# Hydr10n/DirectX-Raytracing-Spheres-Demo

Hardware: AMD Instinct MI355X
Metric: Mrays/s (CastRay-equivalents incl. primaries) at 1920x1080, 8 bounces, 1 spp (higher is better)
Workload: dtype f32

## Files before the change

directx-raytracing-spheres-demo_amd/csrc/pt_api.hip:

```cpp
#include <hip/hip_runtime.h>
#include <rccl/rccl.h>
#include <dlfcn.h>
#include <link.h>

#include <algorithm>
#include <chrono>
#include <cmath>
#include <cstdio>
#include <cstdlib>
#include <cstring>
#include <new>
#include <string>
#include <limits>
#include <vector>

#include "../../include/pt_api.h"
#include "pt_kernels.h"
#include "pt_beam_cache.h"
#include "pt_bloom.h"
#include "pt_nrd.h"
#include "pt_denoise.h"
#include "pt_lbvh.h"
#include "pt_lbvh_gpu.h"

using namespace pt;

namespace {

constexpr uint32_t kMaxLdsBytes = 160u * 1024u;
constexpr uint32_t kSahMaxSpheres = 4096u;
constexpr uint32_t kLdsSceneBudget = 64u * 1024u;

struct EventPair {
    hipEvent_t a, b;
    int kind;
};

}

struct Knobs {
    int split = -1, traverse_blocks_per_cu = -1, fused_threads = -1, no_adaptive_grid = -1, shade_blocks_per_cu = -1, tail_threshold = -1,
        tail_blocks_per_cu = -1, loop_threads = -1, inline2_min_slots = -1, tail_after = -1, seg = -1, loop_use_tail = -1, fuse_loop = -1,
        ray_replacement = -1, dyn_blocks_per_cu = -1, debug_counts = -1, sah = -1, sah_max_spheres = -1, beams = -1, wide = -1, descent = -1, roctx = -1, lane_priority = -1, fused_refit = -1, beam_reach = -1, beam_max_slack_pct = -1, beam_max_margin = -1, beam_share_wgs = -1, refl_beams = -1;
};

struct Lane {
    hipStream_t stream = nullptr;
    hipEvent_t ev_done = nullptr;
    size_t cap_slots = 0;
    RayQueue q[2]{};
    Scratch scratch{};
    bool scratch_spp = false;
    uint32_t* d_counts = nullptr;
    size_t cap_counts = 0;
    uint32_t parity = 0;
    uint32_t* h_counts = nullptr;
    uint32_t* h_prev_counts = nullptr;
    uint32_t* d_prev_counts = nullptr;
    uint64_t prev_signature = 0;
    uint32_t* d_seg_counts = nullptr;
    static constexpr uint32_t kTotals = 10;
    unsigned long long* d_totals = nullptr;
    float4* d_sph = nullptr;
    float4* d_sph_sorted = nullptr;
    float4* d_nodes = nullptr;
    uint32_t* d_refit_flags = nullptr;
    uint32_t* d_refit_hdr = nullptr;
    PtSphere* h_stage = nullptr;
    const float4* d_stage = nullptr;
    hipEvent_t ev_upload = nullptr;
    hipEvent_t ev_poll[4] = {};
    uint32_t scene_n = 0;
    bool scene_private = false;
    uint64_t sph_gen = 0;
    bool needs_refit = false;
    bool upload_pending = false;
    const void* last_out = nullptr;
    const void* last_dn[3] = {};
    const void* last_di[2] = {};
    float4* d_rot = nullptr;
    float4* h_rot_stage = nullptr;
    hipEvent_t ev_rot = nullptr;
    uint64_t rot_gen = 0;
    uint32_t rot_n = 0;
    float4* d_prev_pose = nullptr;
    float4* h_prev_stage = nullptr;
    hipEvent_t ev_prev = nullptr;
    uint32_t prev_cap = 0;
    hipEvent_t ev_gb_in = nullptr;
    void* last_gb[13] = {};
};
constexpr uint32_t kMaxLanes = 8;

struct PtContext {
    int device = 0;
    hipStream_t stream = nullptr;
    bool own_stream = false;
    uint32_t flags = 0;
    uint32_t tile_size = 32;
    uint32_t num_cus = 256;
    Knobs knobs;
    std::string err;
// ... 172 lines not shown
        r.handle = dlopen(name, RTLD_NOW | RTLD_LOCAL);
    }
    if (!r.handle) { r.error = std::string("cannot load librccl.so: ") + dlerror(); return r; }
    auto sym = [&](const char* n) { void* p = dlsym(r.handle, n); if (!p && r.error.empty()) r.error = std::string("librccl.so lacks ") + n; return p; };
    r.GetUniqueId = reinterpret_cast<decltype(r.GetUniqueId)>(sym("ncclGetUniqueId"));
    r.CommInitRank = reinterpret_cast<decltype(r.CommInitRank)>(sym("ncclCommInitRank"));
    r.CommDestroy = reinterpret_cast<decltype(r.CommDestroy)>(sym("ncclCommDestroy"));
    r.GroupStart = reinterpret_cast<decltype(r.GroupStart)>(sym("ncclGroupStart"));
    r.GroupEnd = reinterpret_cast<decltype(r.GroupEnd)>(sym("ncclGroupEnd"));
    r.Send = reinterpret_cast<decltype(r.Send)>(sym("ncclSend"));
    r.Recv = reinterpret_cast<decltype(r.Recv)>(sym("ncclRecv"));
    r.GetErrorString = reinterpret_cast<decltype(r.GetErrorString)>(sym("ncclGetErrorString"));
    if (!r.error.empty()) { dlclose(r.handle); r.handle = nullptr; }
    return r;
}

PtStatus fail(PtContext* ctx, PtStatus st, const std::string& msg)
{
    if (ctx) ctx->err = msg;
    return st;
}

#define PT_HIP(ctx, expr)                                                                              \
    do {                                                                                               \
        hipError_t e_ = (expr);                                                                        \
        if (e_ != hipSuccess) {                                                                        \
            return fail(ctx, e_ == hipErrorOutOfMemory ? PT_ERR_OOM : PT_ERR_HIP,                      \
                        std::string(#expr) + ": " + hipGetErrorString(e_));                            \
        }                                                                                              \
    } while (0)

template <typename T>
void free_dev(T*& p)
{
    if (p) { (void)hipFree(p); p = nullptr; }
}

void free_lane_scene(Lane& L)
{
    free_dev(L.d_sph); free_dev(L.d_sph_sorted); free_dev(L.d_nodes); free_dev(L.d_refit_flags); free_dev(L.d_refit_hdr);
    if (L.h_stage) { (void)hipHostFree(L.h_stage); L.h_stage = nullptr; L.d_stage = nullptr; }
    L.scene_n = 0;
    L.scene_private = false;
    L.upload_pending = false;
    L.needs_refit = false;
}

void free_lane_buffers(Lane& L)
{
    for (auto& q : L.q) { free_dev(q.q0); free_dev(q.q1); free_dev(q.q2); free_dev(q.hit); }
    free_dev(L.scratch.sample_rad); free_dev(L.scratch.radiance); free_dev(L.scratch.primary_hit); free_dev(L.scratch.di); free_dev(L.scratch.primary_cache);
    free_dev(L.scratch.dn.rec); free_dev(L.scratch.dn.di_s);
    L.cap_slots = 0;
    L.scratch_spp = false;
}

PtStatus ensure_buffers(PtContext* c, Lane& L, size_t n_slots, bool need_spp, bool need_hits, size_t n_counts, bool need_di = false)
{
    if (n_slots > L.cap_slots || (need_hits && !L.q[0].hit)) {
        PT_HIP(c, hipStreamSynchronize(L.stream));
        free_lane_buffers(L);
        for (auto& q : L.q) {
            PT_HIP(c, hipMalloc(&q.q0, n_slots * sizeof(float4)));
            PT_HIP(c, hipMalloc(&q.q1, n_slots * sizeof(float4)));
            PT_HIP(c, hipMalloc(&q.q2, n_slots * sizeof(float4)));
            if (need_hits) PT_HIP(c, hipMalloc(&q.hit, n_slots * sizeof(uint2)));
        }
        PT_HIP(c, hipMalloc(&L.scratch.sample_rad, n_slots * sizeof(float4)));
        L.cap_slots = n_slots;
    }
    if (need_di && !L.scratch.di) PT_HIP(c, hipMalloc(&L.scratch.di, L.cap_slots * sizeof(float4)));
    if ((need_spp || need_di) && !L.scratch.primary_hit) PT_HIP(c, hipMalloc(&L.scratch.primary_hit, L.cap_slots * sizeof(uint2)));
    if (need_spp && !L.scratch_spp) {
        PT_HIP(c, hipMalloc(&L.scratch.radiance, L.cap_slots * sizeof(float4)));
        PT_HIP(c, hipMalloc(&L.scratch.primary_cache, L.cap_slots * 3u * sizeof(float4)));
        L.scratch_spp = true;
    }
    if (n_counts > L.cap_counts) {
        free_dev(L.d_counts);
        if (L.h_counts) { (void)hipHostFree(L.h_counts); L.h_counts = nullptr; }
        if (L.h_prev_counts) { (void)hipHostFree(L.h_prev_counts); L.h_prev_counts = nullptr; }
        PT_HIP(c, hipHostMalloc(&L.h_prev_counts, n_counts * sizeof(uint32_t), hipHostMallocMapped));
        std::memset(L.h_prev_counts, 0, n_counts * sizeof(uint32_t));
        PT_HIP(c, hipHostGetDevicePointer(reinterpret_cast<void**>(&L.d_prev_counts), L.h_prev_counts, 0));
        L.prev_signature = 0;
        PT_HIP(c, hipMalloc(&L.d_counts, 4 * n_counts * sizeof(uint32_t)));
        PT_HIP(c, hipMemsetAsync(L.d_counts, 0, 4 * n_counts * sizeof(uint32_t), L.stream));
        PT_HIP(c, hipHostMalloc(&L.h_counts, n_counts * sizeof(uint32_t)));
        L.cap_counts = n_counts;
    }
    return PT_OK;
}

hipError_t sync_all(PtContext* c)
{
    for (uint32_t i = 0; i < c->n_lanes; i++)
        if (c->lanes[i].stream) { hipError_t e = hipStreamSynchronize(c->lanes[i].stream); if (e != hipSuccess) return e; }
    if (c->beam.stream) { hipError_t e = hipStreamSynchronize(c->beam.stream); if (e != hipSuccess) return e; }
    return c->stream ? hipStreamSynchronize(c->stream) : hipSuccess;
}

void free_textures(PtContext* c)
{
    for (auto& img : c->d_tex_images) free_dev(img);
    c->d_tex_images.clear();
    c->tex_dims.clear();
    free_dev(c->d_tex); free_dev(c->d_tex_maps); free_dev(c->d_rot);
    c->has_textures = false;
}

PtStatus sync_lane_rotations(PtContext* c, Lane& L)
{
    if (!c->has_textures || c->rot_gen == c->rot_master_gen || (L.rot_gen == c->rot_gen && L.rot_n == c->n)) return PT_OK;
    const uint32_t n = c->n;
    if (L.rot_n != n) {
        PT_HIP(c, hipStreamSynchronize(L.stream));
        free_dev(L.d_rot);
        if (L.h_rot_stage) { (void)hipHostFree(L.h_rot_stage); L.h_rot_stage = nullptr; }
        PT_HIP(c, hipMalloc(&L.d_rot, (size_t)n * sizeof(float4)));
        PT_HIP(c, hipHostMalloc(&L.h_rot_stage, (size_t)n * sizeof(float4)));
        if (!L.ev_rot) PT_HIP(c, hipEventCreateWithFlags(&L.ev_rot, hipEventDisableTiming));
        L.rot_n = n;
// ... 61 lines not shown
{
    SceneView sv{};
    const bool priv = L && L->scene_private;
    sv.nodes = priv ? L->d_nodes : c->d_nodes;
    sv.wide = priv ? nullptr : c->d_wide;
    sv.sph_sorted = priv ? L->d_sph_sorted : c->d_sph_sorted;
    sv.sorted_id = c->d_leaf_ids ? c->d_leaf_ids : c->d_sorted_id;
    sv.alpha_class = c->d_alpha_class;
    sv.alpha_tested = c->alpha_tested ? 1u : 0u;
    sv.sph = priv ? L->d_sph : c->d_sph;
    sv.mats = c->d_mats;
    sv.n = c->n;
    sv.n_nodes = c->n_nodes;
    sv.stack_depth = stack_entries(c, sv.wide != nullptr);
    sv.descent_cap = c->lds_scene ? 0u : knob_or(c->knobs.descent, 8u);
    sv.lds_scene = c->lds_scene ? 1u : 0u;
    for (int i = 0; i < 4; i++) sv.env[i] = c->sd.EnvironmentLightColor[i];
    if (c->has_textures) { sv.tex = c->d_tex; sv.tex_maps = c->d_tex_maps; sv.rot = (c->rot_gen != c->rot_master_gen && L && L->d_rot && L->rot_gen == c->rot_gen) ? L->d_rot : c->d_rot; }
    sv.env_tex = c->sd.EnvironmentLightTextureDescriptor;
    sv.env_cube = c->sd.IsEnvironmentLightTextureCubeMap ? 1u : 0u;
    for (int r = 0; r < 3; r++)
        for (int k = 0; k < 3; k++) sv.env_xf[3 * r + k] = c->sd.EnvironmentLightTransform[4 * r + k];
    sv.lights = c->d_lights; sv.n_lights = c->n_lights;
    return sv;
}

FrameParams make_frame_params(const PtContext* c)
{
    FrameParams fp{};
    fp.cam = camera_params(c->cam, c->gs.RenderSize[0], c->gs.RenderSize[1]);
    fp.frame_index = c->gs.FrameIndex;
    fp.bounces = c->gs.Bounces;
    fp.spp = c->gs.SamplesPerPixel;
    fp.rr_enabled = c->gs.IsRussianRouletteEnabled ? 1u : 0u;
    fp.throughput_threshold = c->gs.ThroughputThreshold;
    fp.inv_spp = 1.0f / (float)c->gs.SamplesPerPixel;
    fp.di_enabled = (c->gs.IsDIEnabled && c->n_lights > 0) ? 1u : 0u;
    return fp;
}

int env_knob(const char* name)
{
    const char* v = std::getenv(name);
    if (!v || !*v) return -1;
    return (int)std::strtoul(v, nullptr, 10);
}

Knobs read_knobs()
{
    Knobs k;
    k.split = env_knob("PT_SPLIT"); k.traverse_blocks_per_cu = env_knob("PT_TRAVERSE_BLOCKS_PER_CU"); k.fused_threads = env_knob("PT_FUSED_THREADS");
    k.no_adaptive_grid = std::getenv("PT_NO_ADAPTIVE_GRID") ? 1 : -1; k.shade_blocks_per_cu = env_knob("PT_SHADE_BLOCKS_PER_CU");
    k.tail_threshold = env_knob("PT_TAIL_THRESHOLD"); k.tail_blocks_per_cu = env_knob("PT_TAIL_BLOCKS_PER_CU"); k.loop_threads = env_knob("PT_LOOP_THREADS");
    k.inline2_min_slots = env_knob("PT_INLINE2_MIN_SLOTS"); k.tail_after = env_knob("PT_TAIL_AFTER"); k.seg = env_knob("PT_SEG");
    k.loop_use_tail = std::getenv("PT_LOOP_USE_TAIL") ? 1 : -1; k.fuse_loop = env_knob("PT_FUSE_LOOP"); k.beam_reach = env_knob("PT_BEAM_REACH"); k.beam_max_slack_pct = env_knob("PT_BEAM_MAX_SLACK_PCT"); k.beam_max_margin = env_knob("PT_BEAM_MAX_MARGIN"); k.beam_share_wgs = env_knob("PT_BEAM_SHARE_WGS"); k.lane_priority = env_knob("PT_LANE_PRIORITY"); k.fused_refit = env_knob("PT_FUSED_REFIT"); k.ray_replacement = env_knob("PT_RAY_REPLACEMENT");
    k.dyn_blocks_per_cu = env_knob("PT_DYN_BLOCKS_PER_CU"); k.debug_counts = std::getenv("PT_DEBUG_COUNTS") ? 1 : -1; k.sah = env_knob("PT_SAH");
    k.sah_max_spheres = env_knob("PT_SAH_MAX_SPHERES"); k.beams = env_knob("PT_BEAMS"); k.refl_beams = env_knob("PT_REFL_BEAMS"); k.wide = env_knob("PT_WIDE"); k.descent = env_knob("PT_DESCENT"); k.roctx = env_knob("PT_ROCTX");
    return k;
}

EventPair* next_events(PtContext* c, int kind)
{
    if (c->ev_used >= (1u << 20)) return nullptr;
    if (c->ev_used == c->ev_pool.size()) {
        EventPair p{};
        if (hipEventCreate(&p.a) != hipSuccess || hipEventCreate(&p.b) != hipSuccess) return nullptr;
        c->ev_pool.push_back(p);
    }
    EventPair* p = &c->ev_pool[c->ev_used++];
    p->kind = kind;
    return p;
}

uint64_t bytes_per_secondary(bool split) { return split ? 144ull : 96ull; }
uint64_t fixed_bytes(bool split, uint64_t slots, uint64_t pixels, uint64_t spp_paths)
{
    return (split ? 112ull * slots : 0ull) + 16ull * pixels + 48ull * spp_paths;
}

FrameCounters make_counters(const Lane& L, uint32_t parity)
{
    FrameCounters fc{};
    fc.counts = L.d_counts + (size_t)parity * 2 * L.cap_counts;
    fc.fold_counts = L.d_counts + (size_t)(parity ^ 1u) * 2 * L.cap_counts;
    fc.n_counts = (uint32_t)L.cap_counts - 1u;
    fc.tail_rays = L.d_totals + 2 + parity;
    fc.fold_tail = L.d_totals + 2 + (parity ^ 1u);
    fc.totals = L.d_totals;
    fc.host_counts = L.d_prev_counts;
    return fc;
}

hipError_t flush_all_counters(Lane& L)
{
    if (!L.d_counts) return hipSuccess;
    for (uint32_t i = 0; i < 2; i++) {
        const FrameCounters fc = make_counters(L, L.parity ^ 1u ^ i);
        hipError_t e = launch_flush_counters(fc.counts, fc.n_counts, fc.tail_rays, fc.totals, fc.host_counts, L.stream);
        if (e != hipSuccess) return e;
    }
    return hipSuccess;
}

void sum_events(PtContext* c, size_t begin, size_t end, PtStats* stats)
{
    for (size_t i = begin; i < end; i++) {
        float t = 0;
// ... 251 lines not shown
static PtStatus sync_lane_spheres(PtContext* c, Lane& L)
{
    if (c->latest_lane < 0 || L.sph_gen == c->sph_gen) return PT_OK;
    const Lane& src = c->lanes[c->latest_lane];
    if (PtStatus st = stage_spheres_on_lane(c, L, reinterpret_cast<const PtSphere*>(src.h_stage)); st != PT_OK) return st;
    L.sph_gen = c->sph_gen;
    return refit_lane(c, L);
}

static PtStatus check_environment(PtContext* c)
{
    if (const uint32_t env = c->sd.EnvironmentLightTextureDescriptor; env != ~0u) {
        const size_t n_faces = c->sd.IsEnvironmentLightTextureCubeMap ? 6 : 1;
        if (!c->has_textures || (size_t)env + n_faces > c->tex_dims.size())
            return fail(c, PT_ERR_STATE, "SceneData.EnvironmentLightTextureDescriptor names a texture the table of pt_set_textures does not hold (call pt_set_textures after pt_set_scene; a cube map takes six consecutive entries)");
        for (size_t f = 0; f < n_faces; f++)
            if (n_faces == 6 && (c->tex_dims[env + f].first != c->tex_dims[env].first || c->tex_dims[env + f].second != c->tex_dims[env].first))
                return fail(c, PT_ERR_STATE, "SceneData.EnvironmentLightTextureDescriptor: the six faces of a cube map must be square and of one size");
    }
    return PT_OK;
}

struct SuppliedDI {
    const float4* diffuse;
    const float4* specular;
};
PtStatus render_common(PtContext* c, const PixelMap& pm, uint64_t valid_pixels, float4* out, PtStats* stats, const DenoiseOut* dn = nullptr,
                       const SuppliedDI* ext = nullptr)
{
    const RoctxRange range(c, ext ? "pt_render_with_di" : (dn ? "pt_render_denoiser" : (pm.mode == 0 ? "pt_render" : "pt_render_tiles")));
    const uint32_t bounces = c->gs.Bounces, spp = c->gs.SamplesPerPixel;
    if (const PtStatus st = check_environment(c); st != PT_OK) return st;
    const size_t max_iters = (size_t)spp * bounces + 1;
    const size_t wf_cap = spp > 1 ? max_iters : std::min<size_t>(max_iters, 64);
    const bool split = (c->flags & PT_FLAG_SPLIT_KERNELS) || knob_or(c->knobs.split, c->lds_scene ? 0u : 1u) != 0;
    if (traverse_lds_bytes_for(c->n_nodes, c->n, stack_entries(c, c->d_wide != nullptr), c->lds_scene) > kMaxLdsBytes - 9u * 1024u)
        return fail(c, PT_ERR_UNSUPPORTED, "BVH depth needs more traversal-stack LDS than a workgroup can have");
    Lane& L = c->lanes[c->next_lane];
    if (wf_cap + 2 > L.cap_counts && L.cap_counts) {
        PT_HIP(c, flush_all_counters(L));
        PT_HIP(c, hipStreamSynchronize(L.stream));
    }
    const bool di = ext || (c->gs.IsDIEnabled && c->n_lights > 0);
    const bool gb_before = c->gb_frame == c->frames && c->gb_lane == c->next_lane;
    bool lanes_idle = !gb_before || c->gb_lanes_idle;
    for (uint32_t i = 0; i < c->n_lanes && lanes_idle; i++)
        if (!(gb_before && i == c->next_lane) && hipStreamQuery(c->lanes[i].stream) != hipSuccess) { lanes_idle = false; (void)hipGetLastError(); }
    const bool big_frame = c->lds_scene && pm.n_slots >= 1500000u;
    const uint32_t trav_cap = c->num_cus * knob_or(c->knobs.traverse_blocks_per_cu, big_frame ? 2 : 8);
    const uint32_t fused_threads = c->lds_scene ? knob_or(c->knobs.fused_threads, 512) : 256u;
    auto grid_for = [](uint32_t items, uint32_t threads, uint32_t cap) { return std::max(1u, std::min((items + threads - 1) / threads, cap)); };
    const uint32_t primary_grid = grid_for(pm.n_slots, fused_threads, trav_cap);
    const uint32_t primary_batches = (pm.n_slots + fused_threads - 1) / fused_threads;
    const uint32_t seg_cap = (primary_batches + primary_grid - 1) / primary_grid * fused_threads;
    const size_t seg_total = (size_t)primary_grid * seg_cap;
    const bool seg_possible = !split && max_iters > 1 && primary_grid <= kMaxSegs && knob_or(c->knobs.seg, 1u) != 0 && c->knobs.loop_use_tail < 0;
    PtStatus st = ensure_buffers(c, L, split ? pm.n_slots : std::max<size_t>(pm.n_slots, seg_total), spp > 1, split, wf_cap + 2, di);
    if (st != PT_OK) return st;
    if (dn && !L.scratch.dn.rec) PT_HIP(c, hipMalloc(&L.scratch.dn.rec, L.cap_slots * sizeof(float4)));
    if (dn && dn->mode != 1 && di && !L.scratch.dn.di_s) PT_HIP(c, hipMalloc(&L.scratch.dn.di_s, L.cap_slots * sizeof(float4)));
    if ((st = sync_lane_rotations(c, L)) != PT_OK) return st;
    if ((st = sync_lane_spheres(c, L)) != PT_OK) return st;
    if (L.needs_refit && (st = refit_lane(c, L)) != PT_OK) return st;
    c->last_lane = c->next_lane;
    c->next_lane = (c->next_lane + 1) % c->n_lanes;
    c->frames++;
    const uint32_t* beam_lists = nullptr;
    const uint32_t* refl_lists = nullptr;
    BeamJob beam_job{};
    if (!split && !L.scene_private && c->n_nodes > 0 && knob_or(c->knobs.beams, 1u) != 0 && std::fabs(c->cam.Jitter[0]) <= 0.5f && std::fabs(c->cam.Jitter[1]) <= 0.5f) {
        hipEvent_t beam_wait = nullptr;
        if ((st = beam_cache_lookup(c, pm, std::min(primary_grid, knob_or(c->knobs.beam_share_wgs, 128u)) * 64u, &beam_lists, &refl_lists, &beam_wait, &beam_job)) != PT_OK) return st;
        if (beam_wait) PT_HIP(c, hipStreamWaitEvent(L.stream, beam_wait, 0));
    } else {
        c->beam.last_key.clear();
        c->beam.inc.active = false;
    }
    if (L.stream != c->stream) {
        const uint64_t nl = c->n_lanes;
        PT_HIP(c, hipEventRecord(c->ev_in[c->calls % nl], c->stream));
        const hipEvent_t marker = c->ev_in[c->calls >= nl - 1 ? (c->calls - (nl - 1)) % nl : 0];
        if (hipEventQuery(marker) != hipSuccess) {
            (void)hipGetLastError();
            PT_HIP(c, hipStreamWaitEvent(L.stream, marker, 0));
        }
        const void* mine[4] = { out, dn ? dn->diffuse : nullptr, dn ? dn->specular : nullptr, dn ? dn->spec_hit_dist : nullptr };
        bool reused = false;
        for (uint32_t i = 0; i < c->n_lanes && !reused; i++) {
            if (&c->lanes[i] == &L) continue;
            const Lane& o = c->lanes[i];
            const void* theirs[6] = { o.last_out, o.last_dn[0], o.last_dn[1], o.last_dn[2], o.last_di[0], o.last_di[1] };
            for (int a = 0; a < 4 && !reused; a++)
                for (int b = 0; b < 6 && !reused; b++) reused = mine[a] && mine[a] == theirs[b];
        }
        if (ext) reused = true;
        if (reused) PT_HIP(c, hipStreamWaitEvent(L.stream, c->ev_in[c->calls % nl], 0));
        L.last_out = out;
        for (int a = 0; a < 3; a++) L.last_dn[a] = mine[a + 1];
        L.last_di[0] = ext ? ext->diffuse : nullptr;
        L.last_di[1] = ext ? ext->specular : nullptr;
        c->calls++;
    }

    const SceneView sv = make_scene_view(c, &L);
    Scratch scr = L.scratch;
    scr.dn = DenoiseOut{};
    if (dn) {
        scr.dn = *dn;
        scr.dn.rec = L.scratch.dn.rec;
        scr.dn.di_s = L.scratch.dn.di_s;
// ... 18 lines not shown
    const uint32_t shade_cap = c->num_cus * knob_or(c->knobs.shade_blocks_per_cu, 16);
    const bool loop_is_main = spp > 1 && !split && c->knobs.tail_threshold < 0;
    const uint32_t tail_cap = c->num_cus * knob_or(c->knobs.tail_blocks_per_cu, loop_is_main ? 2 : 8);
    const uint32_t trav_threads = traverse_threads(c->lds_scene);
    const uint32_t loop_threads = knob_or(c->knobs.loop_threads, c->lds_scene && (loop_is_main || big_frame) ? 512u : 256u);
    const bool inline2 = !split && spp == 1 && pm.n_slots >= knob_or(c->knobs.inline2_min_slots, 0u);
    const size_t tail_after = knob_or(c->knobs.tail_after, split ? 4 : (inline2 ? 0 : 1));
    const uint32_t tail_threshold = knob_or(c->knobs.tail_threshold, 262144);

    const bool timed = stats != nullptr;
    const size_t ev_begin = c->ev_used;
    if (timed) PT_HIP(c, hipEventRecord(c->ev0, L.stream));

    auto bracket = [&](int kind, auto&& launch) -> hipError_t {
        EventPair* ev = c->profiling ? next_events(c, kind) : nullptr;
        if (ev) (void)hipEventRecord(ev->a, L.stream);
        hipError_t e = launch();
        if (ev) (void)hipEventRecord(ev->b, L.stream);
        return e;
    };
    auto poll = [&](size_t k, bool& empty, bool& go_loop) -> PtStatus {
        empty = false;
        if (loop_is_main) {
            go_loop = true;
        } else if (spp > 1) {
            constexpr size_t kPollLag = 2;
            PT_HIP(c, hipMemcpyAsync(L.h_counts + k + 1, counts + k + 1, sizeof(uint32_t), hipMemcpyDeviceToHost, L.stream));
            PT_HIP(c, hipEventRecord(L.ev_poll[k & 3], L.stream));
            go_loop = k + 2 >= wf_cap;
            if (k >= kPollLag) {
                PT_HIP(c, hipEventSynchronize(L.ev_poll[(k - kPollLag) & 3]));
                const uint32_t v = L.h_counts[k - kPollLag + 1];
                empty = v == 0;
                go_loop = go_loop || v < tail_threshold;
            }
        } else {
            go_loop = k >= tail_after || k + 2 >= wf_cap;
        }
        return PT_OK;
    };

    auto submit = [&]() -> PtStatus {
        if (ext) {
            PT_HIP(c, bracket(1, [&] { return launch_di_gather(pm, ext->diffuse, ext->specular, L.scratch.di, scr.dn.mode > 1 ? scr.dn.di_s : nullptr, L.stream); }));
        } else if (fp.di_enabled && split) {
            const uint32_t di_grid = grid_for(pm.n_slots, trav_threads, trav_cap_wide);
            PT_HIP(c, bracket(1, [&] { return launch_di(sv, pm, fp, L.scratch.di, L.scratch.primary_hit, fc.tail_rays, di_grid, L.stream, scr.dn.mode > 1 ? scr.dn.di_s : nullptr); }));
        }
        if (!split) {
            const bool loop_follows_primary = loop_is_main || (spp == 1 && (tail_after == 0 || wf_cap <= 2));
            const bool seg = loop_follows_primary && seg_possible;
            FrameCounters fc_seg = fc;
            const bool fuse = seg && knob_or(c->knobs.fuse_loop, (pm.n_slots < 400000u || (lanes_idle && spp == 1)) ? 1u : 0u) != 0;
            if (seg) { fc_seg.seg_counts = L.d_seg_counts; fc_seg.n_segs = primary_grid; fc_seg.seg_cap = seg_cap; fc_seg.fuse_loop = fuse ? 1u : 0u; }
            Scratch scratch = scr;
            if (sv.tex_maps || fuse || spp == 1) scratch.primary_cache = nullptr;
            for (size_t k = 0;; k++) {
                const RayQueue& qin = L.q[k & 1];
                const RayQueue& qout = L.q[(k + 1) & 1];
                const bool primary = k == 0;
                bool go_loop = false, empty = false;
                if (k > 0) {
                    if ((st = poll(k - 1, empty, go_loop)) != PT_OK) return st;
                    if (empty) break;
                }
                const bool last_possible = k + 1 >= max_iters;
                const bool loop = (k > 0 && go_loop);
                const uint32_t threads = loop ? loop_threads : fused_threads;
                const uint32_t items = primary ? pm.n_slots : estimate(k);
                const uint32_t cap = loop ? tail_cap : trav_cap;
                if (loop && c->knobs.loop_use_tail >= 0) {
                    PT_HIP(c, launch_tail(sv, pm, fp, qin, scr, out, counts + k, fc.tail_rays, fc.totals, grid_for(items, kTailThreads, tail_cap), L.stream));
                    break;
                }
                PT_HIP(c, bracket(loop ? 3 : (primary ? 0 : 1), [&] {
                    return launch_bounce(sv, pm, fp, qin, qout, scratch, out, counts + k, counts + k + 1, k <= 1 ? fc_seg : fc, primary, loop, inline2, threads,
                                         primary ? primary_grid : grid_for(items, threads, cap), L.stream);
                }));
                if (loop || last_possible || (primary && fuse)) break;
            }
        } else {
            const uint32_t trav_grid = grid_for(pm.n_slots, trav_threads, trav_cap);
            PT_HIP(c, bracket(0, [&] { return launch_primary(sv, pm, fp, L.q[0], scr, out, fc, trav_grid, L.stream); }));
            for (size_t k = 0;; k++) {
                const RayQueue& qin = L.q[k & 1];
                const RayQueue& qout = L.q[(k + 1) & 1];
                PT_HIP(c, bracket(2, [&] { return launch_shade(sv, pm, fp, qin, qout, scr, out, counts + k, counts + k + 1, grid_for(estimate(k), kShadeThreads, shade_cap), L.stream); }));
                if (k + 1 == max_iters) break;
                bool go_loop = false, empty = false;
                if ((st = poll(k, empty, go_loop)) != PT_OK) return st;
                if (empty) break;
                if (go_loop) {
                    PT_HIP(c, bracket(3, [&] { return launch_tail(sv, pm, fp, qout, scr, out, counts + k + 1, fc.tail_rays, fc.totals, grid_for(estimate(k + 1), kTailThreads, tail_cap), L.stream); }));
                    break;
                }
                if (!c->lds_scene && sv.n > 1 && knob_or(c->knobs.ray_replacement, 1)) {
                    uint32_t* cursor = counts + L.cap_counts + k + 1;
                    const uint32_t grid = std::min(grid_for(estimate(k + 1), 256u, c->num_cus * 8u), c->num_cus * knob_or(c->knobs.dyn_blocks_per_cu, 4));
                    PT_HIP(c, bracket(1, [&] { return launch_traverse_dyn(sv, qout, counts + k + 1, cursor, fc.totals, grid, L.stream); }));
                } else {
                    PT_HIP(c, bracket(1, [&] { return launch_traverse(sv, qout, counts + k + 1, grid_for(estimate(k + 1), trav_threads, trav_cap), L.stream); }));
                }
            }
        }
        return PT_OK;
    };
    st = submit();
// ... 1280 lines not shown
```

directx-raytracing-spheres-demo_amd/csrc/pt_device.h:

```cpp
#pragma once

#include <hip/hip_runtime.h>
#include <stdint.h>

#include "pt_bsdf.h"
#include "pt_texture.h"
#include "pt_surface.h"
#include "pt_light.h"

namespace pt {

struct RayQueue {
    float4* q0;
    float4* q1;
    float4* q2;
    uint2* hit;
};

constexpr uint32_t kFlagBounceMask = 0xFFu;
constexpr uint32_t kFlagSampleShift = 8;
constexpr uint32_t kFlagSampleMask = 0xFFFFu;
constexpr uint32_t kFlagDirty = 1u << 24;
constexpr uint32_t kFlagViaTransmission = 1u << 25;
constexpr uint32_t kFlagDnSpecular = 1u << 26;
// ... 73 lines not shown
        const uint32_t bpt_shift = m.ts_shift - 3u;
        const uint32_t b = w >> 6, l = w & 63u;
        const uint32_t lx = ((b & ((1u << bpt_shift) - 1u)) << 3) + (l & 7u), ly = ((b >> bpt_shift) << 3) + (l >> 3);
        uint32_t gt;
        if (m.run == 1u) {
            gt = m.first + k * m.stride;
        } else {
            const uint32_t q = fast_div(k, m.run, m.inv_run, m.exact_div != 0);
            gt = m.first + q * m.stride + (k - q * m.run);
        }
        const uint32_t ty = fast_div(gt, m.tiles_x, m.inv_tiles_x, m.exact_div != 0), tx = gt - ty * m.tiles_x;
        r.px = (tx << m.ts_shift) + lx;
        r.py = (ty << m.ts_shift) + ly;
        r.valid = gt < m.tiles_total && r.px < m.img_w && r.py < m.img_h;
        r.out_index = (k << ts2_shift) + (ly << m.ts_shift) + lx;
    }
    return r;
}

struct BeamJob {
    uint32_t* lists;
    uint32_t first_block, n_blocks;
    float centre[3];
    float slack;
    float right[3], up[3], forward[3];
    float margin_px;
};

struct FrameParams {
    CameraParams cam;
    uint32_t frame_index, bounces, spp, rr_enabled;
    float throughput_threshold;
    float inv_spp;
    uint32_t di_enabled;
    const uint32_t* beam_lists;
    BeamJob beam_job;
    const uint32_t* refl_lists;
};

constexpr uint32_t kDiExternal = 2u;

struct FrameCounters {
    uint32_t* counts;
    uint32_t* fold_counts;
    uint32_t n_counts;
    unsigned long long* tail_rays;
    unsigned long long* fold_tail;
    unsigned long long* totals;
    uint32_t* host_counts;
    uint32_t* seg_counts;
    uint32_t n_segs;
    uint32_t seg_cap;
    uint32_t fuse_loop;
};

constexpr uint32_t kMaxSegs = 2048;

struct DenoiseOut {
    uint32_t mode;
    float4* rec;
    float4* di_s;
    float4* diffuse;
    float4* specular;
    float* spec_hit_dist;
};

struct Scratch {
    float4* sample_rad;
    float4* radiance;
    uint2* primary_hit;
    float4* di;
    float4* primary_cache;
    DenoiseOut dn;
};

}
```

directx-raytracing-spheres-demo_amd/csrc/pt_trace.h:

```cpp
#pragma once

#include "pt_kernels.h"
#include "pt_beam.h"

namespace pt {

__device__ __forceinline__ uint32_t lane_id() { return __builtin_amdgcn_mbcnt_hi(~0u, __builtin_amdgcn_mbcnt_lo(~0u, 0u)); }

__device__ __forceinline__ float fast_rcp(float x) { return __builtin_amdgcn_rcpf(x); }

__device__ __forceinline__ float slab_rcp(float d)
{
    const float kTiny = 1e-30f;
    return fast_rcp(__builtin_fabsf(d) < kTiny ? __builtin_copysignf(kTiny, d) : d);
}

__device__ __forceinline__ void block_atomic_add(unsigned long long* counter, unsigned long long v)
{
    __shared__ unsigned long long s_part[16];
#pragma unroll
    for (int off = 32; off > 0; off >>= 1) v += __shfl_down(v, off, 64);
    __syncthreads();
    if ((threadIdx.x & 63u) == 0) s_part[threadIdx.x >> 6] = v;
    __syncthreads();
// ... 704 lines not shown
template <bool kDn = false>
__device__ __forceinline__ PathState load_path(const RayQueue& q, uint32_t i)
{
    const float4 a = q.q0[i], b = q.q1[i], c = q.q2[i];
    PathState ps;
    ps.o = load3(a); ps.d = load3(b); ps.T = load3(c);
    ps.slot = as_uint(a.w); ps.rng = as_uint(b.w);
    const uint32_t flags = as_uint(c.w);
    ps.bounce = flags & kFlagBounceMask;
    ps.sample = (flags >> kFlagSampleShift) & kFlagSampleMask;
    ps.dirty = (flags & kFlagDirty) != 0;
    ps.via_t = (flags & kFlagViaTransmission) != 0;
    ps.dn_spec = kDn && (flags & kFlagDnSpecular) != 0;
    return ps;
}

template <bool kDn = false>
__device__ __forceinline__ void store_path(const RayQueue& q, uint32_t j, const PathState& ps)
{
    const uint32_t flags = (ps.bounce & kFlagBounceMask) | ((ps.sample & kFlagSampleMask) << kFlagSampleShift) | (ps.dirty ? kFlagDirty : 0u)
                           | (ps.via_t ? kFlagViaTransmission : 0u) | (kDn && ps.dn_spec ? kFlagDnSpecular : 0u);
    q.q0[j] = make_float4(ps.o.x, ps.o.y, ps.o.z, as_float(ps.slot));
    q.q1[j] = make_float4(ps.d.x, ps.d.y, ps.d.z, as_float(ps.rng));
    q.q2[j] = make_float4(ps.T.x, ps.T.y, ps.T.z, as_float(flags));
}

constexpr uint32_t kStaticLdsMargin = (kMaxSegs + 64u) * 4u;

struct BounceArgHead { SceneView sv; PixelMap pm; FrameParams fp; };
template <typename T>
__device__ __forceinline__ T cold_arg(uint32_t offset)
{
    const __attribute__((address_space(4))) char* p = (const __attribute__((address_space(4))) char*)__builtin_amdgcn_kernarg_segment_ptr();
    asm volatile("" : "+s"(p));
    T v;
    __builtin_memcpy(&v, p + offset, sizeof(T));
    return v;
}

template <bool kLds, typename StackT, bool kPrimary, bool kLoop, bool kMulti, bool kTex, bool kInline2, bool kFuse, bool kDI, bool kDn>
__global__ __launch_bounds__(kFusedThreads) __attribute__((amdgpu_waves_per_eu(4, 4))) void bounce_kernel(SceneView sv, PixelMap pm, FrameParams fp, RayQueue qin, RayQueue qout,
                                                               Scratch scratch, float4* __restrict__ out,
                                                               const uint32_t* __restrict__ count_in_ptr, uint32_t* __restrict__ count_out_ptr,
                                                               FrameCounters fc)
{
    constexpr uint32_t kIters = (kPrimary && !kLoop && !kMulti && kInline2) ? 2u : 1u;
    if (kLoop && !kMulti && !kPrimary) __builtin_amdgcn_s_setprio(3);
    extern __shared__ float4 smem[];
    __shared__ uint32_t s_wave_count[kFusedThreads / 64];
    __shared__ uint32_t s_block_base;
    __shared__ uint32_t s_seg_count;
    __shared__ uint32_t s_seg_next;
    __shared__ uint32_t s_loop_next;
    __shared__ uint32_t s_seg_prefix[kMaxSegs + 1];
    __shared__ uint32_t s_refl[2];
    if (kPrimary && blockIdx.x == 0) frame_counters_begin(fc, pm.n_slots);
    const bool seg_out = kPrimary && !kLoop && fc.seg_counts != nullptr;
    const bool seg_in = !kPrimary && kLoop && fc.seg_counts != nullptr;
    uint32_t count;
    if (seg_in) {
        const uint32_t per = (fc.n_segs + blockDim.x - 1u) / blockDim.x;
        const uint32_t first = threadIdx.x * per;
        uint32_t sum = 0;
        for (uint32_t j = 0; j < per; j++) if (first + j < fc.n_segs) sum += fc.seg_counts[first + j];
        uint32_t incl = sum;
#pragma unroll
        for (int off = 1; off < 64; off <<= 1) { const uint32_t v = __shfl_up(incl, off, 64); if ((int)lane_id() >= off) incl += v; }
        if (lane_id() == 63u) s_wave_count[threadIdx.x >> 6] = incl;
        __syncthreads();
        uint32_t base = 0;
        for (uint32_t w = 0; w < (threadIdx.x >> 6); w++) base += s_wave_count[w];
        uint32_t run = base + incl - sum;
        for (uint32_t j = 0; j < per; j++)
            if (first + j < fc.n_segs) { s_seg_prefix[first + j] = run; run += fc.seg_counts[first + j]; }
        if (threadIdx.x == blockDim.x - 1u) s_seg_prefix[fc.n_segs] = base + incl;
        __syncthreads();
        count = s_seg_prefix[fc.n_segs];
        if (blockIdx.x == 0 && threadIdx.x == 0) *const_cast<uint32_t*>(count_in_ptr) = count;
    } else {
        count = kPrimary ? pm.n_slots : *count_in_ptr;
    }
    if (seg_out && threadIdx.x == 0) { s_seg_count = 0; s_seg_next = 0; s_loop_next = 0; }
    if (kIters > 1u && threadIdx.x == 0) { s_refl[0] = 0; s_refl[1] = 0; }
    if (blockIdx.x * blockDim.x >= count) {
        if (seg_out && threadIdx.x == 0) fc.seg_counts[blockIdx.x] = 0;
        return;
    }
    if ((seg_out || kIters > 1u) && !kLds) __syncthreads();
    const float4* nodes = sv.nodes;
    const float4* sph = sv.sph_sorted;
    const uint32_t* ids = sv.sorted_id;
    StackT* stack;
    if (kLds) {
        stage_scene(sv, smem);
        nodes = smem;
        sph = smem + sv.n_nodes * 4u;
        ids = reinterpret_cast<const uint32_t*>(smem + sv.n_nodes * 4u + sv.n);
        stack = reinterpret_cast<StackT*>(reinterpret_cast<char*>(smem) + scene_lds_bytes(sv.n_nodes, sv.n));
    } else {
        stack = reinterpret_cast<StackT*>(smem);
    }
    stack += threadIdx.x;
    const uint32_t lane = lane_id();
    const uint32_t wave = threadIdx.x >> 6;
    uint32_t my_rays = 0;
    if (kPrimary && !kLoop && wave == 0) {
        const BeamJob job = cold_arg<BeamJob>(offsetof(BounceArgHead, fp) + offsetof(FrameParams, beam_job));
        const uint32_t j = blockIdx.x * 64u + lane;
        if (j < job.n_blocks) {
            CameraParams cam_b = cold_arg<CameraParams>(offsetof(BounceArgHead, fp) + offsetof(FrameParams, cam));
            cam_b.Position = make_f3(job.centre[0], job.centre[1], job.centre[2]);
            cam_b.Right = make_f3(job.right[0], job.right[1], job.right[2]);
            cam_b.Up = make_f3(job.up[0], job.up[1], job.up[2]);
            cam_b.Forward = make_f3(job.forward[0], job.forward[1], job.forward[2]);
            beam_walk_block<StackT>(sv, nodes, ids, stack, blockDim.x, cold_arg<PixelMap>(offsetof(BounceArgHead, pm)), cam_b, job.slack, job.margin_px, job.first_block + j, job.lists);
        }
    }
    uint32_t* const cursor = const_cast<uint32_t*>(count_in_ptr) + fc.n_counts + 1u;
    for (uint32_t base = blockIdx.x * blockDim.x;; base += gridDim.x * blockDim.x) {
        uint32_t i;
        if (seg_in) {
            uint32_t b;
            const uint32_t static_end = kMulti ? 0u : gridDim.x * blockDim.x;
            if (!kMulti && base < static_end) {
                b = base + wave * 64u;
            } else {
                if (!kMulti && static_end >= count) break;
                uint32_t v = 0;
                if (lane == 0) v = atomicAdd(cursor, 64u);
                b = static_end + __builtin_amdgcn_readfirstlane(v);
            }
            if (b >= count) break;
            i = b + lane;
        } else if (seg_out) {
            uint32_t w = 0;
            if (lane == 0) w = atomicAdd(&s_seg_next, 1u);
            w = __builtin_amdgcn_readfirstlane(w);
            const uint32_t waves = blockDim.x >> 6;
            const uint32_t b = (blockIdx.x + (w / waves) * gridDim.x) * blockDim.x;
            if (b >= count) break;
            i = b + (w % waves) * 64u + lane;
        } else {
            if (base >= count) break;
            i = base + threadIdx.x;
        }
        bool emit = false;
        PathState ps;
        const uint32_t* beam_rec = nullptr;
        uint32_t beam_count = ~0u;
        if (kPrimary && fp.beam_lists) {
            beam_rec = fp.beam_lists + (size_t)__builtin_amdgcn_readfirstlane(i >> 6) * kBeamRecord;
            beam_count = __builtin_amdgcn_readfirstlane(beam_rec[0]);
        }
        if (i < count) {
            bool live = true;
            float tmin = 0.0f, tmax = kInf;
            if (kPrimary) {
                const PixelMap pm_c = cold_arg<PixelMap>(offsetof(BounceArgHead, pm));
                const PixelRef pr = slot_to_pixel(pm_c, i);
                live = pr.valid;
                ps.slot = i; ps.bounce = 0; ps.sample = 0; ps.dirty = false; ps.via_t = false; ps.dn_spec = false; ps.rng = 0;
                ps.T = make_f3(1.f, 1.f, 1.f);
                ps.o = make_f3(0.f, 0.f, 0.f); ps.d = make_f3(0.f, 0.f, 1.f);
                if (live) {
                    const CameraParams cam_c = cold_arg<CameraParams>(offsetof(BounceArgHead, fp) + offsetof(FrameParams, cam));
                    primary_ray(cam_c, pr.px, pr.py, ps.o, ps.d, tmin, tmax);
                    ps.rng = rng_init(pr.px, pr.py, fp.frame_index);
                } else if (pm_c.mode == 1) {
                    out[pr.out_index] = make_float4(0.f, 0.f, 0.f, 0.f);
                }
            } else if (seg_in) {
                uint32_t lo = 0, hi = fc.n_segs;
                while (hi - lo > 1u) { const uint32_t mid = (lo + hi) >> 1; if (s_seg_prefix[mid] <= i) lo = mid; else hi = mid; }
                ps = load_path<kDn>(qin, lo * fc.seg_cap + (i - s_seg_prefix[lo]));
            } else {
                ps = load_path<kDn>(qin, i);
            }
            constexpr bool kMerged = kLoop && kMulti && !kPrimary;
            if (kMerged) {
                constexpr int kCacheMode = kTex ? 0 : 2;
                bool pending = false;
                for (;;) {
                    float t = 0.0f;
                    uint32_t id = kMissId;
                    if (!pending) closest_hit_any<kLds, StackT, kTex>(sv, nodes, sph, ids, ps.o, ps.d, 0.0f, kInf, stack, blockDim.x, t, id);
                    const int r = shade_step_ex<true, kTex, false, kCacheMode, true, kDn>(sv, pm, fp, scratch, out, ps, t, id, pending);
                    if (r == kShadeDone) break;
                    pending = r == kShadePending;
                    if (!pending) my_rays++;
                }
            } else if (live) {
                bool primary_trace = kPrimary;
// ... 152 lines not shown
```

Measured before the change: 43010.

## Add dynamic global batch cursor for primary-ray segmented scheduling

Replaces the static strided batch assignment in the segmented primary kernel with a per-workgroup chain of batches claimed from a global atomic cursor, so fast workgroups can take more primary batches and load imbalance drops. Segment capacity is doubled to allow up to twice the static share per workgroup, and the second queue buffer is sized separately for that larger segment space. This adds per-batch atomics, LDS spin-waits between waves, and more memory for the segment queue.

```diff
diff --git a/directx-raytracing-spheres-demo_amd/csrc/pt_api.hip b/directx-raytracing-spheres-demo_amd/csrc/pt_api.hip
--- a/directx-raytracing-spheres-demo_amd/csrc/pt_api.hip
+++ b/directx-raytracing-spheres-demo_amd/csrc/pt_api.hip
@@ -41,13 +41,14 @@
 struct Knobs {
     int split = -1, traverse_blocks_per_cu = -1, fused_threads = -1, no_adaptive_grid = -1, shade_blocks_per_cu = -1, tail_threshold = -1,
         tail_blocks_per_cu = -1, loop_threads = -1, inline2_min_slots = -1, tail_after = -1, seg = -1, loop_use_tail = -1, fuse_loop = -1,
-        ray_replacement = -1, dyn_blocks_per_cu = -1, debug_counts = -1, sah = -1, sah_max_spheres = -1, beams = -1, wide = -1, descent = -1, roctx = -1, lane_priority = -1, fused_refit = -1, beam_reach = -1, beam_max_slack_pct = -1, beam_max_margin = -1, beam_share_wgs = -1, refl_beams = -1;
+        ray_replacement = -1, dyn_blocks_per_cu = -1, debug_counts = -1, sah = -1, sah_max_spheres = -1, beams = -1, wide = -1, descent = -1, roctx = -1, lane_priority = -1, fused_refit = -1, beam_reach = -1, beam_max_slack_pct = -1, beam_max_margin = -1, beam_share_wgs = -1, refl_beams = -1, primary_cursor = -1;
 };
 
 struct Lane {
     hipStream_t stream = nullptr;
     hipEvent_t ev_done = nullptr;
     size_t cap_slots = 0;
+    size_t cap_seg = 0;
     RayQueue q[2]{};
     Scratch scratch{};
     bool scratch_spp = false;
@@ -326,22 +327,28 @@
     free_dev(L.scratch.sample_rad); free_dev(L.scratch.radiance); free_dev(L.scratch.primary_hit); free_dev(L.scratch.di); free_dev(L.scratch.primary_cache);
     free_dev(L.scratch.dn.rec); free_dev(L.scratch.dn.di_s);
     L.cap_slots = 0;
+    L.cap_seg = 0;
     L.scratch_spp = false;
 }
 
-PtStatus ensure_buffers(PtContext* c, Lane& L, size_t n_slots, bool need_spp, bool need_hits, size_t n_counts, bool need_di = false)
-{
-    if (n_slots > L.cap_slots || (need_hits && !L.q[0].hit)) {
+PtStatus ensure_buffers(PtContext* c, Lane& L, size_t n_slots, size_t seg_slots, bool need_spp, bool need_hits, size_t n_counts, bool need_di = false)
+{
+    seg_slots = std::max(seg_slots, n_slots);
+    if (n_slots > L.cap_slots || seg_slots > L.cap_seg || (need_hits && !L.q[0].hit)) {
         PT_HIP(c, hipStreamSynchronize(L.stream));
+        n_slots = std::max(n_slots, L.cap_slots);
+        seg_slots = std::max(seg_slots, L.cap_seg);
         free_lane_buffers(L);
         for (auto& q : L.q) {
-            PT_HIP(c, hipMalloc(&q.q0, n_slots * sizeof(float4)));
-            PT_HIP(c, hipMalloc(&q.q1, n_slots * sizeof(float4)));
-            PT_HIP(c, hipMalloc(&q.q2, n_slots * sizeof(float4)));
-            if (need_hits) PT_HIP(c, hipMalloc(&q.hit, n_slots * sizeof(uint2)));
+            const size_t n = &q == &L.q[1] ? seg_slots : n_slots;
+            PT_HIP(c, hipMalloc(&q.q0, n * sizeof(float4)));
+            PT_HIP(c, hipMalloc(&q.q1, n * sizeof(float4)));
+            PT_HIP(c, hipMalloc(&q.q2, n * sizeof(float4)));
+            if (need_hits) PT_HIP(c, hipMalloc(&q.hit, n * sizeof(uint2)));
         }
         PT_HIP(c, hipMalloc(&L.scratch.sample_rad, n_slots * sizeof(float4)));
         L.cap_slots = n_slots;
+        L.cap_seg = seg_slots;
     }
     if (need_di && !L.scratch.di) PT_HIP(c, hipMalloc(&L.scratch.di, L.cap_slots * sizeof(float4)));
     if ((need_spp || need_di) && !L.scratch.primary_hit) PT_HIP(c, hipMalloc(&L.scratch.primary_hit, L.cap_slots * sizeof(uint2)));
@@ -509,7 +516,7 @@
     k.split = env_knob("PT_SPLIT"); k.traverse_blocks_per_cu = env_knob("PT_TRAVERSE_BLOCKS_PER_CU"); k.fused_threads = env_knob("PT_FUSED_THREADS");
     k.no_adaptive_grid = std::getenv("PT_NO_ADAPTIVE_GRID") ? 1 : -1; k.shade_blocks_per_cu = env_knob("PT_SHADE_BLOCKS_PER_CU");
     k.tail_threshold = env_knob("PT_TAIL_THRESHOLD"); k.tail_blocks_per_cu = env_knob("PT_TAIL_BLOCKS_PER_CU"); k.loop_threads = env_knob("PT_LOOP_THREADS");
-    k.inline2_min_slots = env_knob("PT_INLINE2_MIN_SLOTS"); k.tail_after = env_knob("PT_TAIL_AFTER"); k.seg = env_knob("PT_SEG");
+    k.inline2_min_slots = env_knob("PT_INLINE2_MIN_SLOTS"); k.tail_after = env_knob("PT_TAIL_AFTER"); k.seg = env_knob("PT_SEG"); k.primary_cursor = env_knob("PT_PRIMARY_CURSOR");
     k.loop_use_tail = std::getenv("PT_LOOP_USE_TAIL") ? 1 : -1; k.fuse_loop = env_knob("PT_FUSE_LOOP"); k.beam_reach = env_knob("PT_BEAM_REACH"); k.beam_max_slack_pct = env_knob("PT_BEAM_MAX_SLACK_PCT"); k.beam_max_margin = env_knob("PT_BEAM_MAX_MARGIN"); k.beam_share_wgs = env_knob("PT_BEAM_SHARE_WGS"); k.lane_priority = env_knob("PT_LANE_PRIORITY"); k.fused_refit = env_knob("PT_FUSED_REFIT"); k.ray_replacement = env_knob("PT_RAY_REPLACEMENT");
     k.dyn_blocks_per_cu = env_knob("PT_DYN_BLOCKS_PER_CU"); k.debug_counts = std::getenv("PT_DEBUG_COUNTS") ? 1 : -1; k.sah = env_knob("PT_SAH");
     k.sah_max_spheres = env_knob("PT_SAH_MAX_SPHERES"); k.beams = env_knob("PT_BEAMS"); k.refl_beams = env_knob("PT_REFL_BEAMS"); k.wide = env_knob("PT_WIDE"); k.descent = env_knob("PT_DESCENT"); k.roctx = env_knob("PT_ROCTX");
@@ -867,10 +874,13 @@
     auto grid_for = [](uint32_t items, uint32_t threads, uint32_t cap) { return std::max(1u, std::min((items + threads - 1) / threads, cap)); };
     const uint32_t primary_grid = grid_for(pm.n_slots, fused_threads, trav_cap);
     const uint32_t primary_batches = (pm.n_slots + fused_threads - 1) / fused_threads;
-    const uint32_t seg_cap = (primary_batches + primary_grid - 1) / primary_grid * fused_threads;
+    const uint32_t static_share = (primary_batches + primary_grid - 1) / primary_grid;
+    const bool primary_cursor = knob_or(c->knobs.primary_cursor, 1u) != 0 && static_share > 1 && 2 * static_share <= kMaxSegBatches;
+    const uint32_t seg_batches = primary_cursor ? 2 * static_share : static_share;
+    const uint32_t seg_cap = seg_batches * fused_threads;
     const size_t seg_total = (size_t)primary_grid * seg_cap;
     const bool seg_possible = !split && max_iters > 1 && primary_grid <= kMaxSegs && knob_or(c->knobs.seg, 1u) != 0 && c->knobs.loop_use_tail < 0;
-    PtStatus st = ensure_buffers(c, L, split ? pm.n_slots : std::max<size_t>(pm.n_slots, seg_total), spp > 1, split, wf_cap + 2, di);
+    PtStatus st = ensure_buffers(c, L, pm.n_slots, seg_possible ? seg_total : 0, spp > 1, split, wf_cap + 2, di);
     if (st != PT_OK) return st;
     if (dn && !L.scratch.dn.rec) PT_HIP(c, hipMalloc(&L.scratch.dn.rec, L.cap_slots * sizeof(float4)));
     if (dn && dn->mode != 1 && di && !L.scratch.dn.di_s) PT_HIP(c, hipMalloc(&L.scratch.dn.di_s, L.cap_slots * sizeof(float4)));
@@ -995,7 +1005,7 @@
             const bool seg = loop_follows_primary && seg_possible;
             FrameCounters fc_seg = fc;
             const bool fuse = seg && knob_or(c->knobs.fuse_loop, (pm.n_slots < 400000u || (lanes_idle && spp == 1)) ? 1u : 0u) != 0;
-            if (seg) { fc_seg.seg_counts = L.d_seg_counts; fc_seg.n_segs = primary_grid; fc_seg.seg_cap = seg_cap; fc_seg.fuse_loop = fuse ? 1u : 0u; }
+            if (seg) { fc_seg.seg_counts = L.d_seg_counts; fc_seg.n_segs = primary_grid; fc_seg.seg_cap = seg_cap; fc_seg.fuse_loop = fuse ? 1u : 0u; fc_seg.seg_batches = primary_cursor ? seg_batches : 0u; }
             Scratch scratch = scr;
             if (sv.tex_maps || fuse || spp == 1) scratch.primary_cache = nullptr;
             for (size_t k = 0;; k++) {
diff --git a/directx-raytracing-spheres-demo_amd/csrc/pt_device.h b/directx-raytracing-spheres-demo_amd/csrc/pt_device.h
--- a/directx-raytracing-spheres-demo_amd/csrc/pt_device.h
+++ b/directx-raytracing-spheres-demo_amd/csrc/pt_device.h
@@ -149,9 +149,13 @@
     uint32_t n_segs;
     uint32_t seg_cap;
     uint32_t fuse_loop;
+    uint32_t seg_batches;
 };
 
 constexpr uint32_t kMaxSegs = 2048;
+constexpr uint32_t kMaxSegBatches = 254;
+constexpr uint32_t kBatchPending = 0xffffffffu;
+constexpr uint32_t kBatchEnd = 0xfffffffeu;
 
 struct DenoiseOut {
     uint32_t mode;
diff --git a/directx-raytracing-spheres-demo_amd/csrc/pt_trace.h b/directx-raytracing-spheres-demo_amd/csrc/pt_trace.h
--- a/directx-raytracing-spheres-demo_amd/csrc/pt_trace.h
+++ b/directx-raytracing-spheres-demo_amd/csrc/pt_trace.h
@@ -780,6 +780,7 @@
     __shared__ uint32_t s_seg_count;
     __shared__ uint32_t s_seg_next;
     __shared__ uint32_t s_loop_next;
+    __shared__ uint32_t s_batch[kMaxSegBatches + 2];
     __shared__ uint32_t s_seg_prefix[kMaxSegs + 1];
     __shared__ uint32_t s_refl[2];
     if (kPrimary && blockIdx.x == 0) frame_counters_begin(fc, pm.n_slots);
@@ -809,6 +810,9 @@
         count = kPrimary ? pm.n_slots : *count_in_ptr;
     }
     if (seg_out && threadIdx.x == 0) { s_seg_count = 0; s_seg_next = 0; s_loop_next = 0; }
+    const bool seg_cursor = seg_out && fc.seg_batches != 0u;
+    if (seg_cursor)
+        for (uint32_t k = threadIdx.x; k < fc.seg_batches + 2u; k += blockDim.x) s_batch[k] = k ? kBatchPending : blockIdx.x;
     if (kIters > 1u && threadIdx.x == 0) { s_refl[0] = 0; s_refl[1] = 0; }
     if (blockIdx.x * blockDim.x >= count) {
         if (seg_out && threadIdx.x == 0) fc.seg_counts[blockIdx.x] = 0;
@@ -865,7 +869,25 @@
             if (lane == 0) w = atomicAdd(&s_seg_next, 1u);
             w = __builtin_amdgcn_readfirstlane(w);
             const uint32_t waves = blockDim.x >> 6;
-            const uint32_t b = (blockIdx.x + (w / waves) * gridDim.x) * blockDim.x;
+            uint32_t batch;
+            if (seg_cursor) {
+                const uint32_t k = w / waves;
+                while ((batch = __hip_atomic_load(&s_batch[k], __ATOMIC_RELAXED, __HIP_MEMORY_SCOPE_WORKGROUP)) == kBatchPending) __builtin_amdgcn_s_sleep(2);
+                if (w % waves == 0u) {
+                    uint32_t next = kBatchEnd;
+                    if (batch != kBatchEnd && k + 1u < fc.seg_batches) {
+                        uint32_t v = 0;
+                        if (lane == 0) v = atomicAdd(const_cast<uint32_t*>(count_in_ptr) + fc.n_counts + 1u, 1u);
+                        next = gridDim.x + __builtin_amdgcn_readfirstlane(v);
+                        if ((uint64_t)next * blockDim.x >= count) next = kBatchEnd;
+                    }
+                    if (lane == 0) __hip_atomic_store(&s_batch[k + 1u], next, __ATOMIC_RELAXED, __HIP_MEMORY_SCOPE_WORKGROUP);
+                }
+                if (batch == kBatchEnd) break;
+            } else {
+                batch = blockIdx.x + (w / waves) * gridDim.x;
+            }
+            const uint32_t b = batch * blockDim.x;
             if (b >= count) break;
             i = b + (w % waves) * 64u + lane;
         } else {
```

Result: slower. 39890 (-7.2%).
